# SurrealAI/surreal

Measured on AMD Instinct MI355X. Metric: env-steps/sec (learner ingest) PPO 1024 actors×128 steps, 1/2/4/8 MI355X, higher is better.
Workload: dtype f32; 1 GPU; BASELINE configs[4]: PPO synthetic 1024 actors x 128 steps x 376-dim obs per GPU, one learn() per step, batch resident in HBM; mode=adapt, B_per_gpu=1024, n_step=128, obs_dim=376, action_dim=17, epochs=10 policy + 10 value, KL early exit disabled, hip_graph=True, parallelism=dp1, epoch_kernels=fused row-block, graph_segments=False

## Files before the change

include/surreal_amd.h:

```cpp
#ifndef SURREAL_AMD_H
#define SURREAL_AMD_H

#include <stddef.h>
#include <stdint.h>

#ifdef __cplusplus
extern "C" {
#endif

typedef void* smx_stream_t;

enum {
    SMX_OK = 0,
    SMX_E_NULL = -1,
    SMX_E_SHAPE = -2,
    SMX_E_UNSUPPORTED = -3,
    SMX_E_WORKSPACE = -4,
    SMX_E_ALIGN = -5
};

enum { SMX_ACT_NONE = 0, SMX_ACT_RELU = 1, SMX_ACT_TANH = 2 };
enum { SMX_PPO_CLIP = 0, SMX_PPO_ADAPT = 1 };

int smx_abi_version(void);
// ... 24 lines not shown
                              smx_stream_t stream);

int smx_mlp3_fused_exact_zfilter(int32_t on);

size_t smx_mlp3_packed_bytes(int32_t D, int32_t H1, int32_t H2, int32_t OUT);
int smx_mlp3_pack_f32(const smx_mlp3_t* net, float* packed, size_t packed_bytes,
                      smx_stream_t stream);
int smx_mlp3_pack_zstats_f32(const smx_mlp3_t* net, float* packed, size_t packed_bytes,
                             const float* running_sum, const float* running_sumsq, const float* count,
                             int32_t D, float eps, float* mean_out, float* std_out, smx_stream_t stream);
int smx_mlp3_forward_fused_f32(const float* packed, int32_t D, int32_t H1, int32_t H2,
                               int32_t OUT, const float* x_main, const float* x_tail,
                               int64_t G, int32_t T0, int32_t T1, const float* zmean,
                               const float* zstd, float* out, int32_t out_act,
                               smx_stream_t stream);

int smx_linear_f32(const float* A, int32_t lda, int32_t a_kcontig, const float* B,
                   int32_t ldb, int32_t b_kcontig, const float* bias, float* C,
                   int32_t ldc, int32_t M, int32_t N, int32_t K, int32_t act,
                   const float* relu_mask, const int32_t* stop_flag, smx_stream_t stream);

typedef struct smx_linear_job {
    int32_t kind, act;
    const float* A; const float* B; const float* bias; const float* relu_mask;
    float* C; float* dbias;
    int32_t lda, ldb, ldc, a_kcontig, b_kcontig, M, N, K;
    const int32_t* stop_flag;
} smx_linear_job_t;
int smx_linear_multi_f32(const smx_linear_job_t* jobs, int32_t njobs, smx_stream_t stream);

// ... 1044 lines not shown
```

surreal_amd/_lib.py:

```python
import ctypes
import os
from ctypes import (POINTER, Structure, c_char_p, c_double, c_float, c_int32, c_int64, c_size_t,
                    c_uint64, c_void_p)

_HERE = os.path.dirname(os.path.abspath(__file__))
LIB_PATH = os.environ.get('SMX_LIB_PATH') or os.path.join(_HERE, 'libsurreal_amd.so')

SMX_ACT_NONE, SMX_ACT_RELU, SMX_ACT_TANH = 0, 1, 2
SMX_PPO_CLIP, SMX_PPO_ADAPT = 0, 1
SMX_E_UNSUPPORTED = -3
PS_SURR, PS_LOSS, PS_ENTROPY, PS_KL, PS_GRADNORM, PS_LB, PS_ISW, PS_REFBEH, PS_STRIDE = range(9)
VS_LOSS, VS_EXPVAR, VS_GRADNORM = 0, 1, 2
VS_STRIDE = 4


class Mlp3(Structure):
    _fields_ = [('W1', c_void_p), ('b1', c_void_p), ('W2', c_void_p), ('b2', c_void_p),
                ('W3', c_void_p), ('b3', c_void_p),
                ('D', c_int32), ('H1', c_int32), ('H2', c_int32), ('OUT', c_int32)]


class Mlp3Job(Structure):
    _fields_ = [('net', POINTER(Mlp3)), ('x', c_void_p), ('rows', c_int64), ('h1', c_void_p),
                ('h2', c_void_p), ('out', c_void_p), ('out_act', c_int32), ('out_ld', c_int32),
# ... 327 lines not shown
_SIGS = {
    'smx_abi_version': (c_int32, []),
    'smx_error_string': (c_char_p, [c_int32]),
    'smx_zfilter_stats_f32': (c_int32, [_P, _P, _P, c_int32, c_float, _P, _P, _P]),
    'smx_zfilter_forward_f32': (c_int32, [_P, c_int64, c_int64, c_int32, _P, _P, _P, _P]),
    'smx_zfilter_forward_sums_f32': (c_int32, [_P, c_int64, c_int64, c_int32, _P, _P, _P, c_float, _P, _P]),
    'smx_diaggauss_sample_f32': (c_int32, [_P, c_int64, _P, _P, _P, c_int64, c_int64, c_int32, _P,
                                           c_int64, _P, c_int64, _P]),
    'smx_zfilter_update_f32': (c_int32, [_P, c_int64, c_int64, c_int32, _P, _P, _P, c_float, _P]),
    'smx_mlp3_packed_bytes': (c_size_t, [c_int32, c_int32, c_int32, c_int32]),
    'smx_mlp3_pack_f32': (c_int32, [POINTER(Mlp3), _P, c_size_t, _P]),
    'smx_mlp3_pack_zstats_f32': (c_int32, [POINTER(Mlp3), _P, c_size_t, _P, _P, _P, c_int32, c_float, _P, _P, _P]),
    'smx_mlp3_fused_exact_zfilter': (c_int32, [c_int32]),
    'smx_mlp3_forward_fused_f32': (c_int32, [_P, c_int32, c_int32, c_int32, c_int32, _P, _P,
                                             c_int64, c_int32, c_int32, _P, _P, _P, c_int32, _P]),
    'smx_linear_f32': (c_int32, [_P, c_int32, c_int32, _P, c_int32, c_int32, _P, _P, c_int32,
                                 c_int32, c_int32, c_int32, c_int32, _P, _P, _P]),
    'smx_linear_wgrad_f32': (c_int32, [_P, c_int32, _P, c_int32, _P, c_int32, _P, c_int32, c_int32,
                                       c_int32, _P]),
    'smx_mlp3_forward_f32': (c_int32, [POINTER(Mlp3), _P, c_int64, _P, _P, _P, c_int32, _P, _P]),
    'smx_mlp3_forward_multi_f32': (c_int32, [POINTER(Mlp3Job), c_int32, _P]),
    'smx_mlp3_backward_multi_f32': (c_int32, [POINTER(Mlp3Job), c_int32, _P]),
    'smx_mlp3_wgrad_multi_f32': (c_int32, [POINTER(Mlp3Job), c_int32, _P]),
    'smx_epoch_blocks': (c_int32, [c_int64]),
    'smx_epoch_supported': (c_int32, [c_int32, c_int32, c_int32, c_int32]),
    'smx_epoch_packed_floats': (c_int64, [c_int32, c_int32, c_int32, c_int32]),
    'smx_epoch_pack_f32': (c_int32, [POINTER(EpochPack), c_int32, _P]),
    'smx_epoch_prepare_f32': (c_int32, [POINTER(EpochPrep), _P]),
    'smx_epoch_forward_f32': (c_int32, [POINTER(EpochJob), c_int32, POINTER(PpoLosses), _P, c_int64, _P]),
    'smx_epoch_backward_f32': (c_int32, [POINTER(EpochJob), c_int32, POINTER(PpoLosses), _P, c_int64, _P]),
# ... 256 lines not shown
```

surreal_amd/csrc/smx_mlp3_fused.hip:

```cpp
#include "smx_common.h"
#include "smx_mlp3_fused.inc.h"
#include <string.h>

namespace {

constexpr int ROWS_PER_WG = 128;
constexpr int LDS_STRIDE = 36;

inline bool pick_variant(int H1, int H2, int* nt1, int* nt2) {
    if (H1 <= 64 && H2 <= 64) { *nt1 = 2; *nt2 = 2; return true; }
    if (H1 <= 320 && H2 <= 224) { *nt1 = 10; *nt2 = 7; return true; }
    return false;
}

__device__ __forceinline__ float zf(float x, float m, float s) {
    float v = (x - m) / s;
    if (v == v) v = fminf(fmaxf(v, -5.0f), 5.0f);
    return v;
}

__device__ __forceinline__ float relu_f(float v) { return (v < 0.f) ? 0.f : v; }

#define MFMA32(a, b, c) __builtin_amdgcn_mfma_f32_32x32x2f32((a), (b), (c), 0, 0, 0)

// ... 380 lines not shown
                    A.out[myrow * A.OUT + o] = v;
                }
            }
        }
    }
}

struct ZStatsRider {
    const float *rs, *rsq, *cnt;
    float *mean, *stdv;
    int D;
    float eps;
};

__global__ __launch_bounds__(256) void mlp3_pack_kernel(smx_mlp3_t net, float* __restrict__ packed,
                                                        int NT1, int NT2, int KC1, ZStatsRider Z) {
    if (Z.rs) {
        for (int k = blockIdx.x * 256 + threadIdx.x; k < Z.D; k += gridDim.x * 256) {
            const float c = Z.cnt[0];
            const float m = Z.rs[k] / c;
            const float var = Z.rsq[k] / c - m * m;
            float sd = sqrtf(var);
            if (sd == sd) sd = fmaxf(sd, Z.eps);
            Z.mean[k] = m;
            Z.stdv[k] = sd;
        }
    }
    const PackLayout L = pack_layout(NT1, NT2, KC1);
    for (size_t i = (size_t)blockIdx.x * 256 + threadIdx.x; i < L.total; i += (size_t)gridDim.x * 256) {
        float v = 0.f;
        if (i < L.b1) {
// ... 17 lines not shown
            const int f = (int)(i - L.b2);
            if (f < net.H2) v = net.b2[f];
        } else if (i < L.b3) {
            const size_t e = i - L.w3;
            const int kk = (int)(e & 31);
            const size_t rc = e >> 5;
            const int o = (int)(rc & 31), c = (int)(rc >> 5);
            const int k = 32 * c + kk;
            if (o < net.OUT && k < net.H2) v = net.W3[(size_t)o * net.H2 + k];
        } else {
            const int o = (int)(i - L.b3);
            if (o < net.OUT) v = net.b3[o];
        }
        packed[i] = v;
    }
}

template <int NT1, int NT2>
int launch_fused(const FusedArgs& A, hipStream_t st) {
    constexpr int WR = (NT1 > NT2 ? NT1 : NT2) * 32;
    const size_t lds = (size_t)(2 * WR * LDS_STRIDE + 2 * ROWS_PER_WG * LDS_STRIDE + NT1 * 32 +
                                NT2 * 32 + NT2 * 32) * sizeof(float);
    const unsigned grid = (unsigned)((A.total_rows + ROWS_PER_WG - 1) / ROWS_PER_WG);
    const int xmode = (NT1 > 2 && A.xvec && A.D >= 4) ? (A.zmean ? 1 : 2) : 0;
    void (*k)(FusedArgs) = nullptr;
    if (A.OUT == 1) {
        k = xmode == 1 ? mlp3_fused_kernel<NT1, NT2, true, (NT1 > 2 ? 1 : 0)>
          : xmode == 2 ? mlp3_fused_kernel<NT1, NT2, true, (NT1 > 2 ? 2 : 0)>
                       : mlp3_fused_kernel<NT1, NT2, true, 0>;
    } else {
// ... 11 lines not shown

}

static int g_exact_zfilter = 0;
extern "C" int smx_mlp3_fused_exact_zfilter(int32_t on) {
    g_exact_zfilter = on ? 1 : 0;
    return SMX_OK;
}

static long long* g_fused_tbuf = nullptr;
extern "C" void smx_mlp3_fused_debug_tbuf(void* p) { g_fused_tbuf = (long long*)p; }

extern "C" size_t smx_mlp3_packed_bytes(int32_t D, int32_t H1, int32_t H2, int32_t OUT) {
    int nt1, nt2;
    if (D <= 0 || OUT <= 0 || OUT > 32 || !pick_variant(H1, H2, &nt1, &nt2)) return 0;
    return pack_layout(nt1, nt2, (D + 31) / 32).total * sizeof(float);
}

static int pack_launch(const smx_mlp3_t* net, float* packed, size_t packed_bytes, const ZStatsRider& Z,
                       smx_stream_t stream) {
    SMX_REQUIRE(net && packed && net->W1 && net->b1 && net->W2 && net->b2 && net->W3 && net->b3,
                SMX_E_NULL);
    SMX_REQUIRE(net->D > 0 && net->H1 > 0 && net->H2 > 0 && net->OUT > 0, SMX_E_SHAPE);
    int nt1, nt2;
    SMX_REQUIRE(net->OUT <= 32 && pick_variant(net->H1, net->H2, &nt1, &nt2), SMX_E_UNSUPPORTED);
    const int KC1 = (net->D + 31) / 32;
    const PackLayout L = pack_layout(nt1, nt2, KC1);
    SMX_REQUIRE(packed_bytes >= L.total * sizeof(float), SMX_E_WORKSPACE);
    SMX_REQUIRE(((uintptr_t)packed & 15) == 0, SMX_E_ALIGN);
    unsigned blocks = (unsigned)((L.total + 255) / 256);
    if (blocks > 1024) blocks = 1024;
    hipLaunchKernelGGL(mlp3_pack_kernel, dim3(blocks), dim3(256), 0, smx_s(stream), *net, packed, nt1,
                       nt2, KC1, Z);
    SMX_LAUNCH_CHECK();
    return SMX_OK;
}

extern "C" int smx_mlp3_pack_f32(const smx_mlp3_t* net, float* packed, size_t packed_bytes,
                                 smx_stream_t stream) {
    ZStatsRider Z;
    memset(&Z, 0, sizeof(Z));
    return pack_launch(net, packed, packed_bytes, Z, stream);
}

extern "C" int smx_mlp3_pack_zstats_f32(const smx_mlp3_t* net, float* packed, size_t packed_bytes,
                                        const float* running_sum, const float* running_sumsq,
                                        const float* count, int32_t D, float eps, float* mean_out,
                                        float* std_out, smx_stream_t stream) {
    SMX_REQUIRE(running_sum && running_sumsq && count && mean_out && std_out, SMX_E_NULL);
    SMX_REQUIRE(D > 0, SMX_E_SHAPE);
    ZStatsRider Z;
    Z.rs = running_sum; Z.rsq = running_sumsq; Z.cnt = count; Z.mean = mean_out; Z.stdv = std_out;
    Z.D = D; Z.eps = eps;
    return pack_launch(net, packed, packed_bytes, Z, stream);
}

extern "C" int smx_mlp3_forward_fused_f32(const float* packed, int32_t D, int32_t H1, int32_t H2,
                                          int32_t OUT, const float* x_main, const float* x_tail,
                                          int64_t G, int32_t T0, int32_t T1, const float* zmean,
                                          const float* zstd, float* out, int32_t out_act,
                                          smx_stream_t stream) {
    SMX_REQUIRE(packed && x_main && out, SMX_E_NULL);
    SMX_REQUIRE(T1 == 0 || x_tail, SMX_E_NULL);
    SMX_REQUIRE((zmean == nullptr) == (zstd == nullptr), SMX_E_NULL);
    SMX_REQUIRE(G > 0 && T0 > 0 && T1 >= 0 && D > 0 && OUT > 0, SMX_E_SHAPE);
    int nt1, nt2;
    SMX_REQUIRE(OUT <= 32 && pick_variant(H1, H2, &nt1, &nt2), SMX_E_UNSUPPORTED);
    SMX_REQUIRE(((uintptr_t)packed & 15) == 0, SMX_E_ALIGN);
    FusedArgs A;
    A.packed = packed;
    A.x_main = x_main;
    A.x_tail = x_tail ? x_tail : x_main;
    A.zmean = zmean;
    A.zstd = zstd;
    A.out = out;
    A.total_rows = (long)G * (T0 + T1);
    A.T0 = T0;
    A.T1 = T1;
    A.D = D;
    A.OUT = OUT;
    A.KC1 = (D + 31) / 32;
    A.out_act = out_act;
    A.tbuf = g_fused_tbuf;
    A.exp = 0;
    A.h1_out = A.h2_out = nullptr;
    A.H1 = H1; A.H2 = H2; A.out_ld = OUT;
    A.stop = nullptr;
    A.xvec = (D % 4 == 0) && (((uintptr_t)x_main & 15) == 0) &&
             (T1 == 0 || ((uintptr_t)x_tail & 15) == 0) &&
             (zmean == nullptr || ((((uintptr_t)zmean | (uintptr_t)zstd) & 15) == 0));
    if (nt1 == 2) return launch_fused<2, 2>(A, smx_s(stream));
    if (g_exact_zfilter && zmean) A.xvec = 0;
    if (A.xvec) {
        const int rc = smx_rows16_launch(A, H1, H2, smx_s(stream));
        if (rc != SMX_E_UNSUPPORTED) return rc;
    }
    return launch_fused<10, 7>(A, smx_s(stream));
}

extern "C" int32_t smx_mlp3_forward_rows_supported(int32_t D, int32_t H1, int32_t H2, int32_t OUT) {
    int nt1, nt2;
    return D >= 4 && D % 4 == 0 && H1 % 4 == 0 && H2 % 4 == 0 && H1 > 64 && H2 > 64 && OUT >= 1 && OUT <= 32 &&
           pick_variant(H1, H2, &nt1, &nt2) && nt1 > 2;
}

extern "C" int smx_mlp3_forward_rows_f32(const smx_mlp3_t* net, const float* x, int64_t rows, float* h1, float* h2,
                                         float* out, int32_t out_act, int32_t out_ld, float* packed,
                                         size_t packed_bytes, const int32_t* stop_flag, smx_stream_t stream) {
    SMX_REQUIRE(net && x && h1 && h2 && out && packed, SMX_E_NULL);
    SMX_REQUIRE(rows > 0, SMX_E_SHAPE);
    if (!smx_mlp3_forward_rows_supported(net->D, net->H1, net->H2, net->OUT)) return SMX_E_UNSUPPORTED;
    if ((((uintptr_t)x | (uintptr_t)h1 | (uintptr_t)h2) & 15) != 0) return SMX_E_UNSUPPORTED;
    int rc = smx_mlp3_pack_f32(net, packed, packed_bytes, stream);
    if (rc) return rc;
    FusedArgs A;
    A.packed = packed;
    A.x_main = x; A.x_tail = x;
    A.zmean = nullptr; A.zstd = nullptr;
    A.out = out;
    A.total_rows = (long)rows;
    A.T0 = 1; A.T1 = 0;
    A.D = net->D; A.OUT = net->OUT; A.KC1 = (net->D + 31) / 32;
    A.out_act = out_act;
    A.tbuf = nullptr; A.exp = 0; A.xvec = 1;
    A.h1_out = h1; A.h2_out = h2;
    A.H1 = net->H1; A.H2 = net->H2; A.out_ld = out_ld > 0 ? out_ld : net->OUT;
    A.stop = (const int*)stop_flag;
    return smx_rows16_launch(A, net->H1, net->H2, smx_s(stream));
}
```

surreal_amd/csrc/smx_mlp3_fused.inc.h:

```cpp
#pragma once
#include "smx_common.h"

namespace smxf {

struct FusedArgs {
    const float* packed;
    const float* x_main;
    const float* x_tail;
    const float* zmean;
    const float* zstd;
    float* out;
    long total_rows;
    int T0, T1, D, OUT, KC1, out_act, xvec;
    long long* tbuf;
    int exp;
    float* h1_out;
    float* h2_out;
    int H1, H2, out_ld;
    const int* stop;
};

struct PackLayout {
    size_t w1, b1, w2, b2, w3, b3, total;
};

__host__ __device__ inline PackLayout pack_layout(int NT1, int NT2, int KC1) {
    PackLayout L;
    L.w1 = 0;
    L.b1 = L.w1 + (size_t)KC1 * NT1 * 32 * 32;
    L.w2 = L.b1 + (size_t)NT1 * 32;
    L.b2 = L.w2 + (size_t)NT1 * NT2 * 32 * 32;
    L.w3 = L.b2 + (size_t)NT2 * 32;
    L.b3 = L.w3 + (size_t)NT2 * 32 * 32;
    L.total = L.b3 + 32;
    return L;
}

}
using smxf::FusedArgs;
using smxf::PackLayout;
using smxf::pack_layout;

__attribute__((visibility("hidden"))) int smx_rows16_launch(const FusedArgs& A, int H1, int H2, hipStream_t st);
```

surreal_amd/csrc/smx_mlp3_rows16.hip:

```cpp
#include "smx_mlp3_fused.inc.h"

namespace {

constexpr int ROWS16 = 128;
constexpr int LDS16 = 36;
constexpr int NTHR = 512;

#ifdef SMX_FUSED_TIMING
#define TSTAMP(i) do { if (A.tbuf && threadIdx.x == 0) A.tbuf[(size_t)blockIdx.x * 16 + (i)] = (long long)__builtin_readcyclecounter(); } while (0)
#else
#define TSTAMP(i) do { } while (0)
#endif
#define TLOOP(i) do { if (c == 5) TSTAMP(8 + (i)); } while (0)
#ifdef SMX_FUSED_EXP
#define EXP(bit) (SMX_FUSED_EXP & (bit))
#else
#define EXP(bit) 0
#endif
#define MFMA16(a, b, c) __builtin_amdgcn_mfma_f32_16x16x4f32((a), (b), (c), 0, 0, 0)

typedef __amdgpu_buffer_rsrc_t rsrc_t;
typedef unsigned int u32x4 __attribute__((ext_vector_type(4)));

__device__ __forceinline__ rsrc_t make_rsrc(const float* p, unsigned bytes) {
// ... 14 lines not shown
    float v = (x - m) * r;
    if (v == v) v = fminf(fmaxf(v, -5.0f), 5.0f);
    return v;
}
__device__ __forceinline__ void stage_x16(float* dst, float4 v, const float4 zm, const float4 rz, const bool hasz,
                                          const bool ok) {
    const float a = zf16(v.x, zm.x, rz.x), b = zf16(v.y, zm.y, rz.y);
    const float c = zf16(v.z, zm.z, rz.z), d = zf16(v.w, zm.w, rz.w);
    v.x = ok ? (hasz ? a : v.x) : 0.f;
    v.y = ok ? (hasz ? b : v.y) : 0.f;
    v.z = ok ? (hasz ? c : v.z) : 0.f;
    v.w = ok ? (hasz ? d : v.w) : 0.f;
    *reinterpret_cast<float4*>(dst) = v;
}

template <int NT1, int NT2, bool OUT1, bool SAVE>
__global__ __launch_bounds__(NTHR, 1) void mlp3_rows16_kernel(FusedArgs A) {
    constexpr int P1 = (NT1 + 1) / 2, P2 = (NT2 + 1) / 2;
    constexpr int NW1 = (P1 * 32 + 63) / 64, NW2 = (P2 * 32 + 63) / 64;
    constexpr int WR = 64 * (NW1 > NW2 ? NW1 : NW2);
    static_assert(NW1 <= 5 && NW2 <= 4, "staging registers are written out for <= 5 / <= 4 passes");
    extern __shared__ float lds[];
    if (SAVE && A.stop && *A.stop) return;
    TSTAMP(0);
    float* Wb0 = lds;
    float* Wb1 = Wb0 + WR * LDS16;
    float* Xb0 = Wb1 + WR * LDS16;
    float* Xb1 = Xb0 + ROWS16 * LDS16;
    float* b1s = Xb1 + ROWS16 * LDS16;
    float* b2s = b1s + P1 * 32;
    float* w3s = b2s + P2 * 32;
    float* zms = w3s + P2 * 32;
    float* rzl = zms + A.KC1 * 32;

    const int tid = threadIdx.x, lane = tid & 63, wv = tid >> 6;
    const int fm = lane & 15, g = lane >> 4;
    const long row0 = (long)blockIdx.x * ROWS16;
    const PackLayout L = pack_layout(P1, P2, A.KC1);
    const float* W1p = A.packed + L.w1;
    const float* W2p = A.packed + L.w2;
    const float* W3p = A.packed + L.w3;
    const bool hasz = A.zmean != nullptr;
    const rsrc_t rzm = make_rsrc(A.zmean, hasz ? (unsigned)A.D * 4u : 0u);
    const rsrc_t rzs = make_rsrc(A.zstd, hasz ? (unsigned)A.D * 4u : 0u);
// ... 23 lines not shown
        rzl[k] = in ? 1.0f / A.zstd[k] : 1.0f;
    }
    const float b3v = A.packed[L.b3];
    if (OUT1) {
        for (int i = tid; i < P2 * 32; i += NTHR) w3s[i] = W3p[(size_t)(i >> 5) * 1024 + (i & 31)];
    } else {
        if (tid < 32) w3s[tid] = A.packed[L.b3 + tid];
    }

#define SMX_WLD(src, i) (src)[(srow + 64 * (i)) * 8 + sk8]
#define SMX_WST(dst, i, v) *reinterpret_cast<float4*>((dst) + (srow + 64 * (i)) * LDS16 + sk4) = (v)

    f32x4 acc1[NT1];
#pragma unroll
    for (int t = 0; t < NT1; ++t) acc1[t] = f32x4{0.f, 0.f, 0.f, 0.f};

    {
        const float4* wsrc = reinterpret_cast<const float4*>(W1p);
        const int kc = (sk4 < A.D) ? sk4 : A.D - 4;
        const float4 x0 = *reinterpret_cast<const float4*>(xp0 + kc);
        const float4 x1 = *reinterpret_cast<const float4*>(xp1 + kc);
        const float4 zm = ld16(rzm, (unsigned)kc * 4u);
        float4 zs = ld16(rzs, (unsigned)kc * 4u);
        const float4 w0 = SMX_WLD(wsrc, 0), w1 = SMX_WLD(wsrc, 1), w2 = SMX_WLD(wsrc, 2), w3 = SMX_WLD(wsrc, 3);
        float4 w4 = w3;
        if (NW1 > 4) w4 = SMX_WLD(wsrc, 4);
        const float4 rz = make_float4(1.0f / zs.x, 1.0f / zs.y, 1.0f / zs.z, 1.0f / zs.w);
        const bool kin = sk4 < A.D;
        stage_x16(Xb0 + srow * LDS16 + sk4, x0, zm, rz, hasz, xok0 && kin);
        stage_x16(Xb0 + (srow + 64) * LDS16 + sk4, x1, zm, rz, hasz, xok1 && kin);
        SMX_WST(Wb0, 0, w0); SMX_WST(Wb0, 1, w1); SMX_WST(Wb0, 2, w2); SMX_WST(Wb0, 3, w3);
// ... 4 lines not shown

    constexpr int HA = (NT1 + 1) / 2, HB = NT1 - HA;
    constexpr int A1 = HA / 3, A2 = (2 * HA) / 3, B1 = HB / 3, B2 = (2 * HB) / 3;
    float4 fa[HA], fb[HB], bcur, bnxt;
#define SMX_W1(buf) ((buf) + woff)
#define SMX_RD_A(wrow, h, i0, i1)                                                 \
    _Pragma("unroll") for (int t = (i0); t < (i1); ++t)                           \
        fa[t] = *reinterpret_cast<const float4*>((wrow) + t * 16 * LDS16 + 16 * (h));
#define SMX_RD_B(wrow, h, i0, i1)                                                 \
    _Pragma("unroll") for (int t = (i0); t < (i1); ++t)                           \
        fb[t] = *reinterpret_cast<const float4*>((wrow) + (HA + t) * 16 * LDS16 + 16 * (h));
#define SMX_STEP_A(e)                                                             \
    _Pragma("unroll") for (int t = 0; t < HA; ++t) acc1[t] = MFMA16(fa[t].e, bq.e, acc1[t]);
#define SMX_STEP_B(e)                                                             \
    _Pragma("unroll") for (int t = 0; t < HB; ++t) acc1[HA + t] = MFMA16(fb[t].e, bq.e, acc1[HA + t]);
#define SMX_PIN __builtin_amdgcn_sched_barrier(0)
    const int xoff = (wv * 16 + fm) * LDS16 + 4 * g, woff = fm * LDS16 + 4 * g;

    float4 x0, x1, w0, w1, w2, w3, w4;
    const int last = A.KC1 - 1;
    {
        const int cn = 1 < last ? 1 : last;
        const float4* wsrc = reinterpret_cast<const float4*>(W1p + (size_t)cn * P1 * 1024);
        const int k0n = 32 * cn + sk4;
        const int kc = (k0n < A.D) ? k0n : A.D - 4;
        SMX_PIN; w0 = SMX_WLD(wsrc, 0); SMX_PIN; w1 = SMX_WLD(wsrc, 1); SMX_PIN; w2 = SMX_WLD(wsrc, 2); SMX_PIN;
        w3 = SMX_WLD(wsrc, 3); SMX_PIN;
        w4 = w3;
        if (NW1 > 4) w4 = SMX_WLD(wsrc, 4);
        SMX_PIN;
        x0 = *reinterpret_cast<const float4*>(xp0 + kc); SMX_PIN;
        x1 = *reinterpret_cast<const float4*>(xp1 + kc); SMX_PIN;
// ... 81 lines not shown
            SMX_STEP_B(x) SMX_PIN;
            SMX_RD_A(SMX_W1(Wn), 0, A1, A2)
            SMX_PIN;
            SMX_STEP_B(y) SMX_PIN;
            SMX_RD_A(SMX_W1(Wn), 0, A2, HA)
            SMX_PIN;
            SMX_STEP_B(z) SMX_PIN;
            SMX_STEP_B(w) SMX_PIN;
        }
        TLOOP(6);
    }
#undef SMX_STEP_A
#undef SMX_STEP_B
#undef SMX_RD_A
#undef SMX_RD_B
    __syncthreads();

    TSTAMP(2);
#pragma unroll
    for (int t = 0; t < NT1; ++t) {
        const float4 bb = *reinterpret_cast<const float4*>(b1s + 16 * t + 4 * g);
        acc1[t][0] = relu16(acc1[t][0] + bb.x);
        acc1[t][1] = relu16(acc1[t][1] + bb.y);
        acc1[t][2] = relu16(acc1[t][2] + bb.z);
        acc1[t][3] = relu16(acc1[t][3] + bb.w);
    }
    if (SAVE && A.h1_out) {
        const long r = row0 + wv * 16 + fm;
        if (r < A.total_rows) {
            float* dst = A.h1_out + r * (long)A.H1 + 4 * g;
// ... 166 lines not shown
                const int o = (r < 4) ? 4 * g + r : 16 + 4 * g + (r - 4);
                if (o < A.OUT) {
                    float v = ((r < 4) ? acc3[r & 3] : acc3b[r & 3]) + w3s[o];
                    if (A.out_act == SMX_ACT_TANH) v = tanhf(v);
                    else if (A.out_act == SMX_ACT_RELU) v = relu16(v);
                    A.out[myrow * ld + o] = v;
                }
            }
        }
    }
    TSTAMP(5);
#undef SMX_WLD
#undef SMX_WST
}

template <int NT1, int NT2, bool SAVE>
int launch16(const FusedArgs& A, hipStream_t st) {
    constexpr int P1 = (NT1 + 1) / 2, P2 = (NT2 + 1) / 2;
    constexpr int NW1 = (P1 * 32 + 63) / 64, NW2 = (P2 * 32 + 63) / 64;
    constexpr int WR = 64 * (NW1 > NW2 ? NW1 : NW2);
    const size_t lds = (size_t)(2 * WR * LDS16 + 2 * ROWS16 * LDS16 + P1 * 32 + 2 * P2 * 32 + 2 * A.KC1 * 32) * sizeof(float);
    if (lds > 160 * 1024) return SMX_E_UNSUPPORTED;
    const unsigned grid = (unsigned)((A.total_rows + ROWS16 - 1) / ROWS16);
    void (*k)(FusedArgs) = (A.OUT == 1) ? mlp3_rows16_kernel<NT1, NT2, true, SAVE> : mlp3_rows16_kernel<NT1, NT2, false, SAVE>;
    hipError_t e = hipFuncSetAttribute((const void*)k, hipFuncAttributeMaxDynamicSharedMemorySize, (int)lds);
    if (e != hipSuccess) return (int)e;
    hipLaunchKernelGGL(k, dim3(grid), dim3(NTHR), lds, st, A);
    e = hipGetLastError();
    return e == hipSuccess ? SMX_OK : (int)e;
}

}

int smx_rows16_launch(const FusedArgs& A, int H1, int H2, hipStream_t st) {
    const bool save = A.h1_out || A.h2_out;
    if (!A.xvec || A.D < 4 || A.OUT > 32 || H1 <= 64 || H2 <= 64 || H1 > 320 || H2 > 224) return SMX_E_UNSUPPORTED;
    if (save) {
        if ((H1 | H2) & 3) return SMX_E_UNSUPPORTED;
        if (H1 <= 304 && H2 <= 208) return launch16<19, 13, true>(A, st);
        return launch16<20, 14, true>(A, st);
    }
    if (H1 <= 304 && H2 <= 208) return launch16<19, 13, false>(A, st);
    return launch16<20, 14, false>(A, st);
}
```

surreal_amd/kernels.py:

```python
import ctypes

import numpy as np
import torch

from surreal_amd import _lib as L


def _row_stride(view, width):
    assert view.dim() == 2 and view.shape[1] == width and (width == 1 or view.stride(1) == 1), \
        (tuple(view.shape), view.stride())
    return view.stride(0) if view.shape[0] > 1 else max(view.stride(0), width)


def ddpg_rows_ln(kernels):
    return bool(getattr(kernels, 'ddpg_rows_ln', False))


def ddpg_rows_ln_td3(kernels):
    return bool(getattr(kernels, 'ddpg_rows_ln_td3', False))


def ddpg_rows_delay(kernels):
    return bool(getattr(kernels, 'ddpg_rows_delay', False))

# ... 61 lines not shown
                             % (net.D, net.H1, net.H2, net.OUT))
        return nbytes // 4

    def mlp3_pack(self, net, packed):
        L.call('smx_mlp3_pack_f32', ctypes.byref(net.desc), L.ptr(packed), packed.numel() * 4,
               self._st())

    def mlp3_pack_zstats(self, net, packed, zf):
        L.call('smx_mlp3_pack_zstats_f32', ctypes.byref(net.desc), L.ptr(packed), packed.numel() * 4,
               L.ptr(zf.running_sum), L.ptr(zf.running_sumsq), L.ptr(zf.count), zf.running_sum.numel(),
               float(zf.eps), L.ptr(zf._mean), L.ptr(zf._std), self._st())

    def fused_exact_zfilter(self, on):
        L.call('smx_mlp3_fused_exact_zfilter', 1 if on else 0)

    def mlp3_forward_fused(self, packed, net, x_main, x_tail, zmean, zstd, out, act):
        G, T0, D = x_main.shape
        T1 = 0 if x_tail is None else x_tail.shape[1]
        assert x_main.is_contiguous() and (x_tail is None or x_tail.is_contiguous())
        L.call('smx_mlp3_forward_fused_f32', L.ptr(packed), net.D, net.H1, net.H2, net.OUT,
               L.ptr(x_main), L.ptr(x_tail), G, T0, T1, L.ptr(zmean), L.ptr(zstd), L.ptr(out),
               act, self._st())

    FUSED_ROWS_MIN = 24576

    def mlp3_forward(self, net, x, h1, h2, out, act, stop=None, pack=None):
        assert x.is_contiguous()
        if pack is not None and x.shape[0] >= self.FUSED_ROWS_MIN and h1.is_contiguous() and h2.is_contiguous() and \
                L.load().smx_mlp3_forward_rows_supported(net.D, net.H1, net.H2, net.OUT):
            ld = 0 if out.dim() < 2 or out.stride(0) == out.shape[1] else out.stride(0)
            rc = L.load().smx_mlp3_forward_rows_f32(ctypes.byref(net.desc), L.ptr(x), x.shape[0], L.ptr(h1), L.ptr(h2),
                                                    L.ptr(out), act, ld, L.ptr(pack), pack.numel() * 4, L.ptr(stop), self._st())
            if rc != L.SMX_E_UNSUPPORTED:
                L.check(rc, 'smx_mlp3_forward_rows_f32')
                return
        L.call('smx_mlp3_forward_f32', ctypes.byref(net.desc), L.ptr(x), x.shape[0], L.ptr(h1),
               L.ptr(h2), L.ptr(out), act, L.ptr(stop), self._st())
# ... 1423 lines not shown
```

surreal_amd/learner/ppo.py:

```python
import gc
import types

import numpy as np
import torch

from surreal_amd import _lib as L
from surreal_amd import kernels as KN
from surreal_amd.learner.aggregator import MultistepAggregatorWithInfo
from surreal_amd.learner.base import Learner, DeferredStats
from surreal_amd.learner.dist import _SegmentedGraph, _dist_info, setup_peer_exchange
from surreal_amd.model.ppo_net import DiagGauss, PPOModel

EPOCH_PAIR_SPLIT_DEFAULT = True
FOLD_FINAL_STATS_DEFAULT = True
FOLD_EPILOGUE_DEFAULT = True


class LinearWithMinLR(object):

    def __init__(self, initial_lr, num_updates, update_freq=1, min_lr=0.0):
        self.initial_lr = float(initial_lr)
        self.num_updates = max(int(num_updates), 1)
        self.update_freq = max(int(update_freq), 1)
        self.min_lr = float(min_lr)
# ... 114 lines not shown
        self.critic_exp_avg_sq = torch.zeros_like(self.model.critic_flat)
        self.actor_lr_scheduler = LinearWithMinLR(self.lr_actor, num_updates,
                                                  self.lr_update_frequency, self.min_lr)
        self.critic_lr_scheduler = LinearWithMinLR(self.lr_critic, num_updates,
                                                   self.lr_update_frequency, self.min_lr)
        self.aggregator = MultistepAggregatorWithInfo(self.env_config.obs_spec,
                                                      self.env_config.action_spec)
        self.pd = DiagGauss(self.action_dim)
        self.cells = None
        self.filter_rewards = bool(self.use_r_filter) or self.reward_scale != 1.0

        lcfg = self.session_config.learner
        self.use_graph = bool(lcfg.get('use_hip_graph', True)) and self.device != 'cpu' \
            and (self.world_size == 1 or bool(lcfg.get('graph_segments', True)))
        self.fused_epochs = bool(lcfg.get('fused_epochs', True))
        self._ws = None
        self._graphs = {}
        self._ctrl_host = None
        self.trace = None

    def _ensure_ctrl(self, ws):
        vals = [self.actor_lr_scheduler.get_lr()[0], self.critic_lr_scheduler.get_lr()[0],
                getattr(self, 'beta', 0.0), getattr(self, 'eta', 0.0),
                getattr(self, 'clip_epsilon', 0.0), self.kl_target,
                self.actor_gradient_clip_value if self.clip_actor_gradient else 0.0,
                self.critic_gradient_clip_value if self.clip_critic_gradient else 0.0,
                self.actor_regularization, self.critic_regularization]
        if self._ctrl_host != vals:
            ws.ctrl_f[:10].copy_(torch.tensor(vals, dtype=torch.float32))
            self._ctrl_host = vals
# ... 285 lines not shown
        tail = self._enqueue_critic_pass(ws, obs, obs_next)
        if tail is not None:
            self.K.mlp3_forward_multi([tail])
        self._enqueue_gae_from_values(ws, obs, rewards, dones)

    def _enqueue_critic_pass(self, ws, obs, obs_next, filter_tail=True):
        K, m = self.K, self.model
        B, N, D = obs.shape
        zm = zs = None
        if self.use_z_filter:
            K.mlp3_pack_zstats(m.critic, ws.packed, m.z_filter)
            zm, zs = m.z_filter._mean, m.z_filter._std
        else:
            K.mlp3_pack(m.critic, ws.packed)
        if not ws.split_tail:
            K.mlp3_forward_fused(ws.packed, m.critic, obs, obs_next, zm, zs, ws.vals, L.SMX_ACT_NONE)
            return None
        K.mlp3_forward_fused(ws.packed, m.critic, obs, None, zm, zs, ws.vals[:B * N], L.SMX_ACT_NONE)
        if not filter_tail:
            pass
        elif self.use_z_filter:
            K.zfilter_forward(obs_next[:, 0, :], zm, zs, ws.xnext)
        else:
            ws.xnext.copy_(obs_next[:, 0, :])
        return dict(net=m.critic, x=ws.xnext, h1=ws.h1t, h2=ws.h2t, out=ws.vals[B * N:].view(B, 1),
                    act=L.SMX_ACT_NONE)

    def _enqueue_gae_from_values(self, ws, obs, rewards, dones):
        K = self.K
        B, N, D = obs.shape
        vals, tail = (ws.vals[:B * N], ws.vals[B * N:]) if ws.split_tail else (ws.vals, None)
        if ws.merged_tail and self.norm_adv:
            K.gae_norm(vals, rewards, dones, ws.gpow, ws.lpow, self.gamma, self.gamma ** N, B, N, N, ws.adv, ws.ret,
# ... 866 lines not shown
```

Baseline: 126.7 million env-steps/s.

## Use 3-way split-bf16 MFMA for critic forward layer-1 GEMM

```diff
diff --git a/include/surreal_amd.h b/include/surreal_amd.h
--- a/include/surreal_amd.h
+++ b/include/surreal_amd.h
@@ -62,6 +62,10 @@
                                int64_t G, int32_t T0, int32_t T1, const float* zmean,
                                const float* zstd, float* out, int32_t out_act,
                                smx_stream_t stream);
+int smx_mlp3_forward_fused_split_f32(const float* packed, size_t packed_bytes, int32_t split_bf16, int32_t D,
+                                     int32_t H1, int32_t H2, int32_t OUT, const float* x_main,
+                                     const float* x_tail, int64_t G, int32_t T0, int32_t T1, const float* zmean,
+                                     const float* zstd, float* out, int32_t out_act, smx_stream_t stream);
 
 int smx_linear_f32(const float* A, int32_t lda, int32_t a_kcontig, const float* B,
                    int32_t ldb, int32_t b_kcontig, const float* bias, float* C,
diff --git a/surreal_amd/_lib.py b/surreal_amd/_lib.py
--- a/surreal_amd/_lib.py
+++ b/surreal_amd/_lib.py
@@ -365,6 +365,8 @@
     'smx_mlp3_fused_exact_zfilter': (c_int32, [c_int32]),
     'smx_mlp3_forward_fused_f32': (c_int32, [_P, c_int32, c_int32, c_int32, c_int32, _P, _P,
                                              c_int64, c_int32, c_int32, _P, _P, _P, c_int32, _P]),
+    'smx_mlp3_forward_fused_split_f32': (c_int32, [_P, c_size_t, c_int32, c_int32, c_int32, c_int32, c_int32, _P, _P,
+                                                   c_int64, c_int32, c_int32, _P, _P, _P, c_int32, _P]),
     'smx_linear_f32': (c_int32, [_P, c_int32, c_int32, _P, c_int32, c_int32, _P, _P, c_int32,
                                  c_int32, c_int32, c_int32, c_int32, _P, _P, _P]),
     'smx_linear_wgrad_f32': (c_int32, [_P, c_int32, _P, c_int32, _P, c_int32, _P, c_int32, c_int32,
diff --git a/surreal_amd/csrc/smx_mlp3_fused.hip b/surreal_amd/csrc/smx_mlp3_fused.hip
--- a/surreal_amd/csrc/smx_mlp3_fused.hip
+++ b/surreal_amd/csrc/smx_mlp3_fused.hip
@@ -418,7 +418,7 @@
 };
 
 __global__ __launch_bounds__(256) void mlp3_pack_kernel(smx_mlp3_t net, float* __restrict__ packed,
-                                                        int NT1, int NT2, int KC1, ZStatsRider Z) {
+                                                        int NT1, int NT2, int KC1, ZStatsRider Z, int planes) {
     if (Z.rs) {
         for (int k = blockIdx.x * 256 + threadIdx.x; k < Z.D; k += gridDim.x * 256) {
             const float c = Z.cnt[0];
@@ -466,6 +466,24 @@
         }
         packed[i] = v;
     }
+    if (planes) {
+        uint4* dst = reinterpret_cast<uint4*>(packed + L.pl);
+        const size_t items = (size_t)KC1 * NT1 * 2 * 64;
+        for (size_t i = (size_t)blockIdx.x * 256 + threadIdx.x; i < items; i += (size_t)gridDim.x * 256) {
+            const int lane = (int)(i & 63);
+            const size_t ct = i >> 6;
+            const int t = (int)(ct % (size_t)(NT1 * 2)), c = (int)(ct / (size_t)(NT1 * 2));
+            const int f = 16 * t + (lane & 15), k0 = 32 * c + 8 * (lane >> 4);
+            union { __bf16 h[8]; uint4 w; } P[3];
+#pragma unroll
+            for (int j = 0; j < 8; ++j) {
+                const float v = (f < net.H1 && k0 + j < net.D) ? net.W1[(size_t)f * net.D + k0 + j] : 0.f;
+                smxf::split3_bf16(v, P[0].h[j], P[1].h[j], P[2].h[j]);
+            }
+#pragma unroll
+            for (int p = 0; p < 3; ++p) dst[(ct * 3 + p) * 64 + lane] = P[p].w;
+        }
+    }
 }
 
 template <int NT1, int NT2>
@@ -507,7 +525,8 @@
 extern "C" size_t smx_mlp3_packed_bytes(int32_t D, int32_t H1, int32_t H2, int32_t OUT) {
     int nt1, nt2;
     if (D <= 0 || OUT <= 0 || OUT > 32 || !pick_variant(H1, H2, &nt1, &nt2)) return 0;
-    return pack_layout(nt1, nt2, (D + 31) / 32).total * sizeof(float);
+    const PackLayout L = pack_layout(nt1, nt2, (D + 31) / 32);
+    return (nt1 > 2 ? L.total_pl : L.total) * sizeof(float);
 }
 
 static int pack_launch(const smx_mlp3_t* net, float* packed, size_t packed_bytes, const ZStatsRider& Z,
@@ -523,8 +542,9 @@
     SMX_REQUIRE(((uintptr_t)packed & 15) == 0, SMX_E_ALIGN);
     unsigned blocks = (unsigned)((L.total + 255) / 256);
     if (blocks > 1024) blocks = 1024;
+    const int planes = nt1 > 2 && packed_bytes >= L.total_pl * sizeof(float);
     hipLaunchKernelGGL(mlp3_pack_kernel, dim3(blocks), dim3(256), 0, smx_s(stream), *net, packed, nt1,
-                       nt2, KC1, Z);
+                       nt2, KC1, Z, planes);
     SMX_LAUNCH_CHECK();
     return SMX_OK;
 }
@@ -548,11 +568,10 @@
     return pack_launch(net, packed, packed_bytes, Z, stream);
 }
 
-extern "C" int smx_mlp3_forward_fused_f32(const float* packed, int32_t D, int32_t H1, int32_t H2,
-                                          int32_t OUT, const float* x_main, const float* x_tail,
-                                          int64_t G, int32_t T0, int32_t T1, const float* zmean,
-                                          const float* zstd, float* out, int32_t out_act,
-                                          smx_stream_t stream) {
+static int forward_fused(const float* packed, size_t packed_bytes, int32_t split_bf16, int32_t D, int32_t H1,
+                         int32_t H2, int32_t OUT, const float* x_main, const float* x_tail, int64_t G, int32_t T0,
+                         int32_t T1, const float* zmean, const float* zstd, float* out, int32_t out_act,
+                         smx_stream_t stream) {
     SMX_REQUIRE(packed && x_main && out, SMX_E_NULL);
     SMX_REQUIRE(T1 == 0 || x_tail, SMX_E_NULL);
     SMX_REQUIRE((zmean == nullptr) == (zstd == nullptr), SMX_E_NULL);
@@ -579,6 +598,10 @@
     A.h1_out = A.h2_out = nullptr;
     A.H1 = H1; A.H2 = H2; A.out_ld = OUT;
     A.stop = nullptr;
+    {
+        const PackLayout L = pack_layout(nt1, nt2, A.KC1);
+        A.planes = (split_bf16 && !g_exact_zfilter && nt1 > 2 && packed_bytes >= L.total_pl * sizeof(float)) ? packed + L.pl : nullptr;
+    }
     A.xvec = (D % 4 == 0) && (((uintptr_t)x_main & 15) == 0) &&
              (T1 == 0 || ((uintptr_t)x_tail & 15) == 0) &&
              (zmean == nullptr || ((((uintptr_t)zmean | (uintptr_t)zstd) & 15) == 0));
@@ -589,6 +612,23 @@
         if (rc != SMX_E_UNSUPPORTED) return rc;
     }
     return launch_fused<10, 7>(A, smx_s(stream));
+}
+
+extern "C" int smx_mlp3_forward_fused_f32(const float* packed, int32_t D, int32_t H1, int32_t H2,
+                                          int32_t OUT, const float* x_main, const float* x_tail,
+                                          int64_t G, int32_t T0, int32_t T1, const float* zmean,
+                                          const float* zstd, float* out, int32_t out_act,
+                                          smx_stream_t stream) {
+    return forward_fused(packed, 0, 0, D, H1, H2, OUT, x_main, x_tail, G, T0, T1, zmean, zstd, out, out_act, stream);
+}
+
+extern "C" int smx_mlp3_forward_fused_split_f32(const float* packed, size_t packed_bytes, int32_t split_bf16,
+                                                int32_t D, int32_t H1, int32_t H2, int32_t OUT,
+                                                const float* x_main, const float* x_tail, int64_t G, int32_t T0,
+                                                int32_t T1, const float* zmean, const float* zstd, float* out,
+                                                int32_t out_act, smx_stream_t stream) {
+    return forward_fused(packed, packed_bytes, split_bf16, D, H1, H2, OUT, x_main, x_tail, G, T0, T1, zmean, zstd,
+                         out, out_act, stream);
 }
 
 extern "C" int32_t smx_mlp3_forward_rows_supported(int32_t D, int32_t H1, int32_t H2, int32_t OUT) {
@@ -617,6 +657,7 @@
     A.out_act = out_act;
     A.tbuf = nullptr; A.exp = 0; A.xvec = 1;
     A.h1_out = h1; A.h2_out = h2;
+    A.planes = nullptr;
     A.H1 = net->H1; A.H2 = net->H2; A.out_ld = out_ld > 0 ? out_ld : net->OUT;
     A.stop = (const int*)stop_flag;
     return smx_rows16_launch(A, net->H1, net->H2, smx_s(stream));
diff --git a/surreal_amd/csrc/smx_mlp3_fused.inc.h b/surreal_amd/csrc/smx_mlp3_fused.inc.h
--- a/surreal_amd/csrc/smx_mlp3_fused.inc.h
+++ b/surreal_amd/csrc/smx_mlp3_fused.inc.h
@@ -18,11 +18,21 @@
     float* h2_out;
     int H1, H2, out_ld;
     const int* stop;
+    const void* planes;
 };
 
 struct PackLayout {
     size_t w1, b1, w2, b2, w3, b3, total;
+    size_t pl, total_pl;
 };
+
+__host__ __device__ inline void split3_bf16(float v, __bf16& hi, __bf16& mid, __bf16& lo) {
+    hi = (__bf16)v;
+    const float r1 = v - (float)hi;
+    mid = (__bf16)r1;
+    const float r2 = r1 - (float)mid;
+    lo = (__bf16)r2;
+}
 
 __host__ __device__ inline PackLayout pack_layout(int NT1, int NT2, int KC1) {
     PackLayout L;
@@ -33,6 +43,8 @@
     L.w3 = L.b2 + (size_t)NT2 * 32;
     L.b3 = L.w3 + (size_t)NT2 * 32 * 32;
     L.total = L.b3 + 32;
+    L.pl = L.total;
+    L.total_pl = L.pl + (size_t)KC1 * NT1 * 2 * 3 * 64 * 4;
     return L;
 }
 
diff --git a/surreal_amd/csrc/smx_mlp3_rows16.hip b/surreal_amd/csrc/smx_mlp3_rows16.hip
--- a/surreal_amd/csrc/smx_mlp3_rows16.hip
+++ b/surreal_amd/csrc/smx_mlp3_rows16.hip
@@ -52,20 +52,51 @@
     *reinterpret_cast<float4*>(dst) = v;
 }
 
-template <int NT1, int NT2, bool OUT1, bool SAVE>
+template <int NT1, int NT2, bool SPLIT1>
+struct Lds16 {
+    static constexpr int P1 = (NT1 + 1) / 2, P2 = (NT2 + 1) / 2;
+    static constexpr int NW1 = (P1 * 32 + 63) / 64, NW2 = (P2 * 32 + 63) / 64;
+    static constexpr int WR = 64 * (NW1 > NW2 ? NW1 : NW2);
+    static constexpr int WBF = SPLIT1 ? (NT1 * 768 > 64 * NW2 * LDS16 ? NT1 * 768 : 64 * NW2 * LDS16) : WR * LDS16;
+    static constexpr int XBF = SPLIT1 ? 0 : ROWS16 * LDS16;
+};
+
+typedef __bf16 bf16x8 __attribute__((ext_vector_type(8)));
+#define MFMAB(a, b, c) __builtin_amdgcn_mfma_f32_16x16x32_bf16((a), (b), (c), 0, 0, 0)
+
+__device__ __forceinline__ void split_x16(bf16x8 (&pl)[3], const float4 a, const float4 b, const float* zms,
+                                          const float* rzl, const int k, const bool hasz, const bool oka,
+                                          const bool okb) {
+    const float4 ma = *reinterpret_cast<const float4*>(zms + k), mb = *reinterpret_cast<const float4*>(zms + k + 4);
+    const float4 ra = *reinterpret_cast<const float4*>(rzl + k), rb = *reinterpret_cast<const float4*>(rzl + k + 4);
+    const float raw[8] = {a.x, a.y, a.z, a.w, b.x, b.y, b.z, b.w};
+    const float m[8] = {ma.x, ma.y, ma.z, ma.w, mb.x, mb.y, mb.z, mb.w};
+    const float r[8] = {ra.x, ra.y, ra.z, ra.w, rb.x, rb.y, rb.z, rb.w};
+#pragma unroll
+    for (int j = 0; j < 8; ++j) {
+        const float z = zf16(raw[j], m[j], r[j]);
+        const float v = ((j < 4) ? oka : okb) ? (hasz ? z : raw[j]) : 0.f;
+        __bf16 h, mi, lo;
+        smxf::split3_bf16(v, h, mi, lo);
+        pl[0][j] = h; pl[1][j] = mi; pl[2][j] = lo;
+    }
+}
+
+template <int NT1, int NT2, bool OUT1, bool SAVE, bool SPLIT1>
 __global__ __launch_bounds__(NTHR, 1) void mlp3_rows16_kernel(FusedArgs A) {
     constexpr int P1 = (NT1 + 1) / 2, P2 = (NT2 + 1) / 2;
     constexpr int NW1 = (P1 * 32 + 63) / 64, NW2 = (P2 * 32 + 63) / 64;
-    constexpr int WR = 64 * (NW1 > NW2 ? NW1 : NW2);
+    constexpr int WBF = Lds16<NT1, NT2, SPLIT1>::WBF, XBF = Lds16<NT1, NT2, SPLIT1>::XBF;
     static_assert(NW1 <= 5 && NW2 <= 4, "staging registers are written out for <= 5 / <= 4 passes");
+    static_assert(!(SPLIT1 && SAVE), "the stem instantiations stay on fp32 MFMA");
     extern __shared__ float lds[];
     if (SAVE && A.stop && *A.stop) return;
     TSTAMP(0);
     float* Wb0 = lds;
-    float* Wb1 = Wb0 + WR * LDS16;
-    float* Xb0 = Wb1 + WR * LDS16;
-    float* Xb1 = Xb0 + ROWS16 * LDS16;
-    float* b1s = Xb1 + ROWS16 * LDS16;
+    float* Wb1 = Wb0 + WBF;
+    float* Xb0 = Wb1 + WBF;
+    float* Xb1 = Xb0 + XBF;
+    float* b1s = Xb1 + XBF;
     float* b2s = b1s + P1 * 32;
     float* w3s = b2s + P2 * 32;
     float* zms = w3s + P2 * 32;
@@ -119,7 +150,119 @@
     f32x4 acc1[NT1];
 #pragma unroll
     for (int t = 0; t < NT1; ++t) acc1[t] = f32x4{0.f, 0.f, 0.f, 0.f};
-
+    const int woff = fm * LDS16 + 4 * g;
+#define SMX_PIN __builtin_amdgcn_sched_barrier(0)
+
+    if constexpr (SPLIT1) {
+    constexpr int NWORD = NT1 * 192, NPS = (NWORD + NTHR - 1) / NTHR, CW = P1 * 2 * 192;
+    static_assert(NPS == 8, "staging registers are written out for 8 passes");
+    const uint4* PL = reinterpret_cast<const uint4*>(A.planes);
+    uint4* Pb0 = reinterpret_cast<uint4*>(Wb0);
+    uint4* Pb1 = reinterpret_cast<uint4*>(Wb1);
+    const int last = A.KC1 - 1;
+    const float* xq;
+    bool xokq;
+    {
+        const int T = A.T0 + A.T1;
+        const long r = row0 + wv * 16 + fm;
+        xokq = r < A.total_rows;
+        const long rr = xokq ? r : 0;
+        const long gq = rr / T;
+        const int tt = (int)(rr - gq * T);
+        xq = (tt < A.T0) ? A.x_main + (gq * A.T0 + tt) * (long)A.D : A.x_tail + (gq * A.T1 + (tt - A.T0)) * (long)A.D;
+    }
+#define SMX_PIDX(i) ((tid + NTHR * (i) < NWORD) ? tid + NTHR * (i) : NWORD - 1)
+#define SMX_PLD(src, i) (src)[SMX_PIDX(i)]
+#define SMX_PST(dst, i, v) do { if (tid + NTHR * (i) < NWORD) (dst)[tid + NTHR * (i)] = (v); } while (0)
+#define SMX_XLD(c_, va, vb, ka, kb)                                                                        \
+    do {                                                                                                   \
+        const int k0_ = 32 * (c_) + 8 * g;                                                                 \
+        ka = k0_ < A.D; kb = k0_ + 4 < A.D;                                                                \
+        va = *reinterpret_cast<const float4*>(xq + (ka ? k0_ : A.D - 4));                                  \
+        vb = *reinterpret_cast<const float4*>(xq + (kb ? k0_ + 4 : A.D - 4));                              \
+    } while (0)
+    uint4 s0, s1, s2, s3, s4, s5, s6, s7;
+    float4 xa, xb;
+    bool ka, kb;
+    bf16x8 bx[3], bn[3];
+    {
+        SMX_XLD(0, xa, xb, ka, kb);
+        s0 = SMX_PLD(PL, 0); s1 = SMX_PLD(PL, 1); s2 = SMX_PLD(PL, 2); s3 = SMX_PLD(PL, 3);
+        s4 = SMX_PLD(PL, 4); s5 = SMX_PLD(PL, 5); s6 = SMX_PLD(PL, 6); s7 = SMX_PLD(PL, 7);
+        SMX_PST(Pb0, 0, s0); SMX_PST(Pb0, 1, s1); SMX_PST(Pb0, 2, s2); SMX_PST(Pb0, 3, s3);
+        SMX_PST(Pb0, 4, s4); SMX_PST(Pb0, 5, s5); SMX_PST(Pb0, 6, s6); SMX_PST(Pb0, 7, s7);
+    }
+    __syncthreads();
+    TSTAMP(1);
+    split_x16(bx, xa, xb, zms, rzl, 8 * g, hasz, xokq && ka, xokq && kb);
+    {
+        const int cn = 1 < last ? 1 : last;
+        const uint4* src = PL + (size_t)cn * CW;
+        SMX_PIN; s0 = SMX_PLD(src, 0); SMX_PIN; s1 = SMX_PLD(src, 1); SMX_PIN; s2 = SMX_PLD(src, 2); SMX_PIN;
+        s3 = SMX_PLD(src, 3); SMX_PIN; s4 = SMX_PLD(src, 4); SMX_PIN; s5 = SMX_PLD(src, 5); SMX_PIN;
+        s6 = SMX_PLD(src, 6); SMX_PIN; s7 = SMX_PLD(src, 7); SMX_PIN;
+        SMX_XLD(cn, xa, xb, ka, kb); SMX_PIN;
+    }
+    bf16x8 fr[3][3];
+#define SMX_RDF(slot, buf, t_)                                                                             \
+    _Pragma("unroll") for (int p_ = 0; p_ < 3; ++p_)                                                       \
+        fr[slot][p_] = *reinterpret_cast<const bf16x8*>((buf) + ((t_) * 3 + p_) * 64 + lane);
+    SMX_RDF(0, Pb0, 0)
+    SMX_RDF(1, Pb0, 1)
+    for (int c = 0; c < A.KC1; ++c) {
+        const uint4* Pc = (c & 1) ? Pb1 : Pb0;
+        uint4* Pn = (c & 1) ? Pb0 : Pb1;
+        const int cn = (c + 1 < A.KC1) ? c + 1 : c;
+        const int c2 = (c + 2 < A.KC1) ? c + 2 : last;
+        const uint4* src = PL + (size_t)c2 * CW;
+        SMX_PIN;
+#pragma unroll
+        for (int t = 0; t < NT1; ++t) {
+            if (t == NT1 - 2) __syncthreads();
+            if (t + 2 < NT1) { SMX_RDF((t + 2) % 3, Pc, t + 2) } else { SMX_RDF((t + 2) % 3, Pn, t + 2 - NT1) }
+            SMX_PIN;
+            {
+                const bf16x8 wh = fr[t % 3][0], wm = fr[t % 3][1], wl = fr[t % 3][2];
+                f32x4 a = acc1[t];
+                a = MFMAB(wl, bx[0], a);
+                a = MFMAB(wh, bx[2], a);
+                a = MFMAB(wm, bx[1], a);
+                a = MFMAB(wm, bx[0], a);
+                a = MFMAB(wh, bx[1], a);
+                a = MFMAB(wh, bx[0], a);
+                acc1[t] = a;
+            }
+            SMX_PIN;
+            if (t == 1) { SMX_PST(Pn, 0, s0); s0 = SMX_PLD(src, 0); }
+            if (t == 2) { SMX_PST(Pn, 1, s1); s1 = SMX_PLD(src, 1); }
+            if (t == 3) { SMX_PST(Pn, 2, s2); s2 = SMX_PLD(src, 2); }
+            if (t == 4) { SMX_PST(Pn, 3, s3); s3 = SMX_PLD(src, 3); }
+            if (t == 5) { SMX_PST(Pn, 4, s4); s4 = SMX_PLD(src, 4); }
+            if (t == 6) { SMX_PST(Pn, 5, s5); s5 = SMX_PLD(src, 5); }
+            if (t == 7) { SMX_PST(Pn, 6, s6); s6 = SMX_PLD(src, 6); }
+            if (t == 8) { SMX_PST(Pn, 7, s7); s7 = SMX_PLD(src, 7); }
+            if (t == 0) {
+                asm volatile("" : "+v"(xa.x), "+v"(xa.y), "+v"(xa.z), "+v"(xa.w), "+v"(xb.x), "+v"(xb.y), "+v"(xb.z), "+v"(xb.w));
+                split_x16(bn, xa, xb, zms, rzl, 32 * cn + 8 * g, hasz, xokq && ka, xokq && kb);
+                SMX_XLD(c2, xa, xb, ka, kb);
+            }
+            SMX_PIN;
+        }
+        bx[0] = bn[0]; bx[1] = bn[1]; bx[2] = bn[2];
+        {
+            bf16x8 q0[3], q1[3];
+#pragma unroll
+            for (int p = 0; p < 3; ++p) { q0[p] = fr[NT1 % 3][p]; q1[p] = fr[(NT1 + 1) % 3][p]; }
+#pragma unroll
+            for (int p = 0; p < 3; ++p) { fr[0][p] = q0[p]; fr[1][p] = q1[p]; }
+        }
+    }
+#undef SMX_RDF
+#undef SMX_XLD
+#undef SMX_PST
+#undef SMX_PLD
+#undef SMX_PIDX
+    } else {
     {
         const float4* wsrc = reinterpret_cast<const float4*>(W1p);
         const int kc = (sk4 < A.D) ? sk4 : A.D - 4;
@@ -154,8 +297,7 @@
     _Pragma("unroll") for (int t = 0; t < HA; ++t) acc1[t] = MFMA16(fa[t].e, bq.e, acc1[t]);
 #define SMX_STEP_B(e)                                                             \
     _Pragma("unroll") for (int t = 0; t < HB; ++t) acc1[HA + t] = MFMA16(fb[t].e, bq.e, acc1[HA + t]);
-#define SMX_PIN __builtin_amdgcn_sched_barrier(0)
-    const int xoff = (wv * 16 + fm) * LDS16 + 4 * g, woff = fm * LDS16 + 4 * g;
+    const int xoff = (wv * 16 + fm) * LDS16 + 4 * g;
 
     float4 x0, x1, w0, w1, w2, w3, w4;
     const int last = A.KC1 - 1;
@@ -267,6 +409,7 @@
 #undef SMX_STEP_B
 #undef SMX_RD_A
 #undef SMX_RD_B
+    }
     __syncthreads();
 
     TSTAMP(2);
@@ -463,15 +606,15 @@
 #undef SMX_WST
 }
 
-template <int NT1, int NT2, bool SAVE>
+template <int NT1, int NT2, bool SAVE, bool SPLIT1>
 int launch16(const FusedArgs& A, hipStream_t st) {
     constexpr int P1 = (NT1 + 1) / 2, P2 = (NT2 + 1) / 2;
-    constexpr int NW1 = (P1 * 32 + 63) / 64, NW2 = (P2 * 32 + 63) / 64;
-    constexpr int WR = 64 * (NW1 > NW2 ? NW1 : NW2);
-    const size_t lds = (size_t)(2 * WR * LDS16 + 2 * ROWS16 * LDS16 + P1 * 32 + 2 * P2 * 32 + 2 * A.KC1 * 32) * sizeof(float);
+    constexpr int WBF = Lds16<NT1, NT2, SPLIT1>::WBF, XBF = Lds16<NT1, NT2, SPLIT1>::XBF;
+    const size_t lds = (size_t)(2 * WBF + 2 * XBF + P1 * 32 + 2 * P2 * 32 + 2 * A.KC1 * 32) * sizeof(float);
     if (lds > 160 * 1024) return SMX_E_UNSUPPORTED;
     const unsigned grid = (unsigned)((A.total_rows + ROWS16 - 1) / ROWS16);
-    void (*k)(FusedArgs) = (A.OUT == 1) ? mlp3_rows16_kernel<NT1, NT2, true, SAVE> : mlp3_rows16_kernel<NT1, NT2, false, SAVE>;
+    void (*k)(FusedArgs) = (A.OUT == 1) ? mlp3_rows16_kernel<NT1, NT2, true, SAVE, SPLIT1>
+                                        : mlp3_rows16_kernel<NT1, NT2, false, SAVE, SPLIT1>;
     hipError_t e = hipFuncSetAttribute((const void*)k, hipFuncAttributeMaxDynamicSharedMemorySize, (int)lds);
     if (e != hipSuccess) return (int)e;
     hipLaunchKernelGGL(k, dim3(grid), dim3(NTHR), lds, st, A);
@@ -486,9 +629,13 @@
     if (!A.xvec || A.D < 4 || A.OUT > 32 || H1 <= 64 || H2 <= 64 || H1 > 320 || H2 > 224) return SMX_E_UNSUPPORTED;
     if (save) {
         if ((H1 | H2) & 3) return SMX_E_UNSUPPORTED;
-        if (H1 <= 304 && H2 <= 208) return launch16<19, 13, true>(A, st);
-        return launch16<20, 14, true>(A, st);
-    }
-    if (H1 <= 304 && H2 <= 208) return launch16<19, 13, false>(A, st);
-    return launch16<20, 14, false>(A, st);
-}
+        if (H1 <= 304 && H2 <= 208) return launch16<19, 13, true, false>(A, st);
+        return launch16<20, 14, true, false>(A, st);
+    }
+    if (A.planes) {
+        const int rc = (H1 <= 304 && H2 <= 208) ? launch16<19, 13, false, true>(A, st) : launch16<20, 14, false, true>(A, st);
+        if (rc != SMX_E_UNSUPPORTED) return rc;
+    }
+    if (H1 <= 304 && H2 <= 208) return launch16<19, 13, false, false>(A, st);
+    return launch16<20, 14, false, false>(A, st);
+}
diff --git a/surreal_amd/kernels.py b/surreal_amd/kernels.py
--- a/surreal_amd/kernels.py
+++ b/surreal_amd/kernels.py
@@ -99,13 +99,13 @@
     def fused_exact_zfilter(self, on):
         L.call('smx_mlp3_fused_exact_zfilter', 1 if on else 0)
 
-    def mlp3_forward_fused(self, packed, net, x_main, x_tail, zmean, zstd, out, act):
+    def mlp3_forward_fused(self, packed, net, x_main, x_tail, zmean, zstd, out, act, split_bf16=True):
         G, T0, D = x_main.shape
         T1 = 0 if x_tail is None else x_tail.shape[1]
         assert x_main.is_contiguous() and (x_tail is None or x_tail.is_contiguous())
-        L.call('smx_mlp3_forward_fused_f32', L.ptr(packed), net.D, net.H1, net.H2, net.OUT,
-               L.ptr(x_main), L.ptr(x_tail), G, T0, T1, L.ptr(zmean), L.ptr(zstd), L.ptr(out),
-               act, self._st())
+        L.call('smx_mlp3_forward_fused_split_f32', L.ptr(packed), packed.numel() * 4, 1 if split_bf16 else 0,
+               net.D, net.H1, net.H2, net.OUT, L.ptr(x_main), L.ptr(x_tail), G, T0, T1, L.ptr(zmean),
+               L.ptr(zstd), L.ptr(out), act, self._st())
 
     FUSED_ROWS_MIN = 24576
 
diff --git a/surreal_amd/learner/ppo.py b/surreal_amd/learner/ppo.py
--- a/surreal_amd/learner/ppo.py
+++ b/surreal_amd/learner/ppo.py
@@ -152,6 +152,8 @@
         self.use_graph = bool(lcfg.get('use_hip_graph', True)) and self.device != 'cpu' \
             and (self.world_size == 1 or bool(lcfg.get('graph_segments', True)))
         self.fused_epochs = bool(lcfg.get('fused_epochs', True))
+        self.critic_split_bf16 = bool(lcfg.get('critic_split_bf16', True))
+        self._critic_kw = {} if self.critic_split_bf16 else {'split_bf16': False}
         self._ws = None
         self._graphs = {}
         self._ctrl_host = None
@@ -467,9 +469,11 @@
         else:
             K.mlp3_pack(m.critic, ws.packed)
         if not ws.split_tail:
-            K.mlp3_forward_fused(ws.packed, m.critic, obs, obs_next, zm, zs, ws.vals, L.SMX_ACT_NONE)
+            K.mlp3_forward_fused(ws.packed, m.critic, obs, obs_next, zm, zs, ws.vals, L.SMX_ACT_NONE,
+                                 **self._critic_kw)
             return None
-        K.mlp3_forward_fused(ws.packed, m.critic, obs, None, zm, zs, ws.vals[:B * N], L.SMX_ACT_NONE)
+        K.mlp3_forward_fused(ws.packed, m.critic, obs, None, zm, zs, ws.vals[:B * N], L.SMX_ACT_NONE,
+                             **self._critic_kw)
         if not filter_tail:
             pass
         elif self.use_z_filter:
```

Result: faster. 137.8 million env-steps/s, median of 6 (+8.7%).
